# sriramelango/optimized-diffusion-model

Hardware: AMD Instinct MI355X
Metric: trajectories/sec (1000-step PC sampler, NCSN++ [1,9,9], bs=128/GPU) (higher is better)
Workload: dtype f32; 1 GPU; NCSN++ nf=64 ch_mult=[1,2,2] on [128,1,9,9] per GPU, 1000-step reflected PC sampler (predictor euler_maruyama, corrector none), classifier-free guidance on (2B-sample forwards), fp32; global_batch=128, num_scales=1000, score_evals_per_traj=999, parallelism=single GPU

## Files before the change

optimized-diffusion-model_amd/csrc/misc_kernels.h:

```cpp
#pragma once
#include "common.h"

struct PackJob {
    const float* src;
    float* dst;
    int Cin, Cout;
    int Kpad;
    int Npad;
    int n_off;
    int ntap;
    long s_co, s_ci, s_t;
    int kind;
    const float* src2;
    int col_il;
};

__global__ __launch_bounds__(RDMI_THREADS) void pack_kernel(const PackJob* __restrict__ jobs) {
    const PackJob j = jobs[blockIdx.y];
    const int stride = gridDim.x * RDMI_THREADS;
    if (j.kind == 1) {
        for (int i = blockIdx.x * RDMI_THREADS + threadIdx.x; i < j.Cout; i += stride) j.dst[j.n_off + i] = j.src[i];
        return;
    }
    if (j.kind == 4) {
        for (int i = blockIdx.x * RDMI_THREADS + threadIdx.x; i < j.Cout; i += stride) {
            float acc = 0.f;
            for (int k = 0; k < j.Cin; ++k) acc = fmaf(j.src[k], j.src2[(long)k * j.Cout + i], acc);
            j.dst[j.n_off + i] = acc;
        }
        return;
    }
    if (j.kind == 2) {
        const int ncol = (j.Cout + 15) & ~15;
        bf16_t* d16 = reinterpret_cast<bf16_t*>(j.dst);
        const long total = (long)j.ntap * (j.Kpad >> 5) * ncol * 32;
        for (long i = blockIdx.x * RDMI_THREADS + threadIdx.x; i < total; i += stride) {
            const int kk = (int)(i & 31);
            long r = i >> 5;
            const int co = (int)(r % ncol); r /= ncol;
            const int ch = (int)(r % (j.Kpad >> 5));
            const int t = (int)(r / (j.Kpad >> 5));
            const int ci = ch * 32 + kk;
            float v = 0.f;
            if (co < j.Cout && ci < j.Cin) v = j.src[co * j.s_co + ci * j.s_ci + t * j.s_t];
            int pos = j.n_off + co;
            if (j.col_il > 1) { const int F = j.col_il, w = pos % (16 * F); pos = pos - w + (w % F) * 16 + w / F; }
            d16[(((long)t * (j.Kpad >> 5) + ch) * j.Npad + pos) * 32 + kk] = f2bf(v);
        }
        return;
    }
    const int ncol = (j.Cout + 15) & ~15;
    const long total = (long)j.ntap * (j.Kpad >> 4) * ncol * 16;
    for (long i = blockIdx.x * RDMI_THREADS + threadIdx.x; i < total; i += stride) {
        const int kk = (int)(i & 15);
        long r = i >> 4;
        const int co = (int)(r % ncol); r /= ncol;
        const int ch = (int)(r % (j.Kpad >> 4));
        const int t = (int)(r / (j.Kpad >> 4));
        const int ci = ch * 16 + kk;
        float v = 0.f;
        if (co < j.Cout && ci < j.Cin) {
            if (j.kind == 3) {
                for (int k = 0; k < j.Cout; ++k) v = fmaf(j.src[(long)ci * j.s_ci + k * j.s_co], j.src2[(long)k * j.Cout + co], v);
            } else if (j.kind == 5) {
                const int py = t >> 3, px = (t >> 2) & 1, ty = (t >> 1) & 1, tx = t & 1;
                const int ky0 = ty * (1 + py), ky1 = ky0 + 1 + (py != ty);
                const int kx0 = tx * (1 + px), kx1 = kx0 + 1 + (px != tx);
                const float* const s = j.src + co * j.s_co + ci * j.s_ci;
                bool first = true;
                for (int ky = ky0; ky < ky1; ++ky)
                    for (int kx = kx0; kx < kx1; ++kx) {
                        const float wv = s[(ky * 3 + kx) * j.s_t];
                        v = first ? wv : v + wv;
                        first = false;
                    }
            } else v = j.src[co * j.s_co + ci * j.s_ci + t * j.s_t];
        }
        j.dst[(((long)t * (j.Kpad >> 4) + ch) * j.Npad + j.n_off + co) * 16 + kk] = v;
    }
}

struct LinArgs {
    const float* X; int ldx;
    const float* W; int Npad;
    const float* bias;
    float* Y; int ldy;
    int M, N, K;
    int pre;
    const float* fourW; int nfour; int x_mod; int t_is_time; float smin, ratio;
    int use_scalar; float t_scalar;
    const float* labels; const float* Wl; const float* bl; int ncls; int label_rows;
    int row_div;
};

__device__ __forceinline__ float sigma_of(float v, int t_is_time, float smin, float ratio) {
    return t_is_time ? smin * powf(ratio, v) : v;
}

template <int NT, int UNR = 4>
__global__ __launch_bounds__(RDMI_THREADS) void linear_mfma_kernel(LinArgs a) {
    const int tid = threadIdx.x, lane = tid & 63, wave = tid >> 6;
    const int lrow = lane & 15, kq = lane >> 4;
    const int row = blockIdx.x * 16 + lrow;
    int col[NT], lcol[NT];
#pragma unroll
    for (int t = 0; t < NT; ++t) {
        col[t] = blockIdx.y * (64 * NT) + (wave * NT + t) * 16 + lrow;
        lcol[t] = min(col[t], a.Npad - 16 + lrow);
    }
    f32x4 acc[NT];
#pragma unroll
    for (int t = 0; t < NT; ++t) acc[t] = f32x4{0.f, 0.f, 0.f, 0.f};
    float ls = 0.f;
    if (a.pre == 2 && row < a.M) ls = logf(sigma_of(a.use_scalar ? a.t_scalar : a.X[row % a.x_mod], a.t_is_time, a.smin, a.ratio));
#pragma unroll UNR
    for (int ch = 0; ch < (a.K >> 4); ++ch) {
// ... 373 lines not shown
```

optimized-diffusion-model_amd/csrc/rdmi.hip:

```cpp
#include <hip/hip_runtime.h>

#include <algorithm>
#include <cmath>
#include <cstdarg>
#include <cstdio>
#include <cstdlib>
#include <cstring>
#include <climits>
#include <map>
#include <memory>
#include <stdexcept>
#include <string>
#include <vector>

#include "../../include/rdmi.h"
#include "attn_kernel.h"
#include "conv_kernel.h"
#include "misc_kernels.h"
#include "unet_kernel.h"
#include "bwd_kernels.h"
#include "opt_kernels.h"
#include "ode_kernels.h"
#include "tiled_kernels.h"

// ... 246 lines not shown
    L.mid_ch = in_ch;
    std::vector<int> sk(L.skip_ch.rbegin(), L.skip_ch.rend());
    int u = 0, k = 0;
    for (int i = a.n_levels - 1; i >= 0; --i) {
        const int out_ch = a.nf * a.ch_mult[i];
        for (int j = 0; j < a.num_res_blocks + 1; ++j) {
            L.up.push_back({"up_blocks." + std::to_string(u), in_ch + sk[k++], out_ch, (a.attn_levels >> i & 1) != 0, i});
            in_ch = out_ch;
            ++u;
        }
    }
    return L;
}

void build_params(rdmi_ctx* c, const Layout& L) {
    const rdmi_arch& a = c->arch;
    add_param(c, "time_embed.W", {a.nf});
    add_param(c, "time_mlp.0.weight", {c->temb, 2 * a.nf});
    add_param(c, "time_mlp.0.bias", {c->temb});
    add_param(c, "time_mlp.2.weight", {c->temb, c->temb});
    add_param(c, "time_mlp.2.bias", {c->temb});
    if (a.conditional) {
        add_param(c, "label_emb.weight", {c->temb, a.num_classes});
        add_param(c, "label_emb.bias", {c->temb});
    }
    add_conv_p(c, "input_conv", a.channels, a.nf);
    for (auto& b : L.down) add_resblock_p(c, b.name, b.cin, b.cout);
    for (size_t i = 0; i < L.down.size(); ++i)
        if (L.down[i].attn) add_attn_p(c, "down_attn." + std::to_string(i), L.down[i].cout);
    {
        int ch = a.nf;
        for (int i = 0; i < a.n_levels; ++i) {
            ch = a.nf * a.ch_mult[i];
            if (i != a.n_levels - 1) add_conv_p(c, "downsample." + std::to_string(i) + ".Conv_0", ch, ch);
        }
    }
    add_resblock_p(c, "mid_block1", L.mid_ch, L.mid_ch);
    add_resblock_p(c, "mid_block2", L.mid_ch, L.mid_ch);
    for (auto& b : L.up) add_resblock_p(c, b.name, b.cin, b.cout);
    for (size_t i = 0; i < L.up.size(); ++i)
        if (L.up[i].attn) add_attn_p(c, "up_attn." + std::to_string(i), L.up[i].cout);
    for (int k = 0, i = a.n_levels - 1; i >= 1; --i, ++k) {
        const int ch = a.nf * a.ch_mult[i];
        add_conv_p(c, "upsample." + std::to_string(k) + ".Conv_0", ch, ch);
    }
    add_gn(c, "out_norm", a.nf * a.ch_mult[0]);
    add_conv_p(c, "out_conv", a.nf * a.ch_mult[0], a.channels);
}

inline bool up_fold_shape_ok(int Hs, int Ws, int Cin, int Cout) {
    return std::getenv("RDMI_NO_UP_FOLD") == nullptr && Hs * Ws == 16 && Cin == Cout && Cin % 128 == 0;
}

struct Builder {
    rdmi_ctx* c;
    std::vector<int> ints;
    size_t wf = 0;

    int new_tensor(const std::string& name, int C, int H, int W) {
        Tensor t;
        t.name = name; t.C = C; t.H = H; t.W = W;
        t.def = (int)c->ops.size();
        c->tensors.push_back(t);
        return (int)c->tensors.size() - 1;
    }
    void use(int t) { if (t >= 0) c->tensors[t].last = (int)c->ops.size(); }

    size_t alloc_w(size_t n) { size_t o = wf; wf += (n + 63) & ~(size_t)63; return o; }

    void job_pack(const std::string& pname, size_t dst_off, int Cin, int Cout, int Kpad, int Npad, int n_off, int ntap,
                  long s_co, long s_ci, long s_t) {
        PackJob j{};
        j.dst = reinterpret_cast<float*>(dst_off);
        j.Cin = Cin; j.Cout = Cout; j.Kpad = Kpad; j.Npad = Npad; j.n_off = n_off; j.ntap = ntap;
        j.s_co = s_co; j.s_ci = s_ci; j.s_t = s_t; j.kind = 0;
        c->jobs.push_back(j);
        c->job_param.push_back(c->pindex.at(pname));
    }
    void job_copy(const std::string& pname, size_t dst_off, int n, int n_off) {
        PackJob j{};
        j.dst = reinterpret_cast<float*>(dst_off);
        j.Cout = n; j.n_off = n_off; j.kind = 1;
        c->jobs.push_back(j);
        c->job_param.push_back(c->pindex.at(pname));
    }
    size_t pack_conv(const std::string& pre, int cin, int cout) {
        const int Kp = pad16(cin), Np = pad16(cout);
        size_t o = alloc_w((size_t)9 * Kp * Np);
        job_pack(pre + ".weight", o, cin, cout, Kp, Np, 0, 9, (long)cin * 9, 9, 1);
        c->wmap[pre] = o;
        return o;
    }
    size_t pack_nin(const std::string& pre, int cin, int cout) {
        const int Kp = pad16(cin), Np = pad16(cout);
        size_t o = alloc_w((size_t)Kp * Np);
        job_pack(pre + ".W", o, cin, cout, Kp, Np, 0, 1, 1, cout, 0);
        c->wmap[pre] = o;
        return o;
    }

    static std::vector<int> nearest_map(int Hs, int Ws, int Hd, int Wd) {
        std::vector<int> m((size_t)Hd * Wd);
        for (int y = 0; y < Hd; ++y)
            for (int x = 0; x < Wd; ++x) {
                int sy = std::min((int)std::floor(y * ((float)Hs / Hd)), Hs - 1);
                int sx = std::min((int)std::floor(x * ((float)Ws / Wd)), Ws - 1);
// ... 67 lines not shown
    }

    int add_attn(const std::string& name, int tin, int C, int H, int W, int* err) {
        Op op;
        op.kind = OP_ATTN;
        op.name = name;
        if (C != 64 || H * W > 96) { *err = fail("attention %s: only C=64, H*W<=96 is built (got C=%d, L=%d)", name.c_str(), C, H * W); return -1; }
        AttnArgs& a = op.attn;
        a.L = H * W; a.Lpad = pad16(a.L); a.G = std::min(C / 4, 32);
        a.eps = 1e-6f; a.scale = 1.0f / std::sqrt((float)C); a.out_scale = (float)(1.0 / std::sqrt(2.0));
        op.tA = tin;
        op.w_off = alloc_w((size_t)3 * C * C);
        for (int i = 0; i < 3; ++i) {
            PackJob j{};
            j.dst = reinterpret_cast<float*>(op.w_off + (size_t)i * C * C);
            j.Cin = C; j.Cout = C; j.Kpad = C; j.Npad = C; j.n_off = 0; j.ntap = 1; j.s_co = 1; j.s_ci = C; j.s_t = 0; j.kind = 0;
            c->jobs.push_back(j);
            c->job_param.push_back(c->pindex.at(name + ".NIN_" + std::to_string(i) + ".W"));
        }
        c->wmap[name + ".qkv"] = op.w_off;
        {
            const size_t o3 = alloc_w((size_t)3 * C * C);
            for (int i = 0; i < 3; ++i) {
                PackJob j{};
                j.dst = reinterpret_cast<float*>(o3);
                j.Cin = C; j.Cout = C; j.Kpad = C; j.Npad = 3 * C; j.n_off = i * C; j.ntap = 1; j.s_co = 1; j.s_ci = C; j.s_t = 0; j.kind = 0;
                c->jobs.push_back(j);
                c->job_param.push_back(c->pindex.at(name + ".NIN_" + std::to_string(i) + ".W"));
            }
            c->wmap[name + ".qkv3"] = o3;
        }
        {
            const size_t o3 = alloc_w((size_t)3 * C * C);
            for (int i = 0; i < 3; ++i) {
                PackJob j{};
                j.dst = reinterpret_cast<float*>(o3);
                j.Cin = C; j.Cout = C; j.Kpad = C; j.Npad = 3 * C; j.n_off = i * C; j.ntap = 1; j.s_co = 1; j.s_ci = C; j.s_t = 0; j.kind = i == 2 ? 3 : 0;
                c->jobs.push_back(j);
                c->job_param.push_back(c->pindex.at(name + ".NIN_" + std::to_string(i) + ".W"));
                c->job_param2.resize(c->jobs.size(), -1);
                if (i == 2) c->job_param2.back() = c->pindex.at(name + ".NIN_3.W");
            }
            c->wmap[name + ".qkv3f"] = o3;
            const size_t ob = alloc_w((size_t)3 * C);
            c->wmap[name + ".bqkvf"] = ob;
            for (int i = 0; i < 2; ++i) job_copy(name + ".NIN_" + std::to_string(i) + ".b", ob, C, i * C);
            PackJob j{};
            j.dst = reinterpret_cast<float*>(ob);
            j.Cin = C; j.Cout = C; j.n_off = 2 * C; j.kind = 4;
            c->jobs.push_back(j);
            c->job_param.push_back(c->pindex.at(name + ".NIN_2.b"));
            c->job_param2.resize(c->jobs.size(), -1);
            c->job_param2.back() = c->pindex.at(name + ".NIN_3.W");
        }
        op.bqkv_off = alloc_w((size_t)3 * C);
        c->wmap[name + ".bqkv"] = op.bqkv_off;
        for (int i = 0; i < 3; ++i) job_copy(name + ".NIN_" + std::to_string(i) + ".b", op.bqkv_off, C, i * C);
        op.w3_off = pack_nin(name + ".NIN_3", C, C);
        op.p_b3 = name + ".NIN_3.b";
        op.p_gamma = name + ".GroupNorm_0.weight"; op.p_beta = name + ".GroupNorm_0.bias";
        op.flops_per_sample = 2.0 * (4.0 * a.L * C * C + 2.0 * a.L * a.L * C);
        op.attn_C = C; op.attn_H = H; op.attn_W = W;
        use(tin);
        const int out = new_tensor(name, C, H, W);
        op.out_tensor = out;
        c->ops.push_back(op);
        return out;
    }
};

int add_resblock(Builder& b, const std::string& name, int tA, int tB, int CA, int CB, int Ha, int Wa, int H, int W,
                 int cout, int dense_off, int* err) {
    ConvSpec s0;
    s0.name = name + ".Conv_0";
    s0.tA = tA; s0.tB = tB; s0.CA = CA; s0.CB = CB; s0.Ha = Ha; s0.Wa = Wa; s0.Hv = H; s0.Wv = W;
    s0.gn = name + ".GroupNorm_0"; s0.conv = name + ".Conv_0";
    s0.Ho = H; s0.Wo = W; s0.Cout = cout; s0.dense_off = dense_off;
    const int h1 = b.add_conv(s0, err);
    if (*err) return -1;
    ConvSpec s1;
    s1.name = name;
    s1.tA = h1; s1.CA = cout; s1.Ha = H; s1.Wa = W; s1.Hv = H; s1.Wv = W;
    s1.gn = name + ".GroupNorm_1"; s1.conv = name + ".Conv_1";
    s1.Ho = H; s1.Wo = W; s1.Cout = cout;
    s1.scale = (float)(1.0 / std::sqrt(2.0));
    s1.dropout = true;
    if (CA + CB != cout) {
        s1.tScA = tA; s1.tScB = tB; s1.CscA = CA; s1.CscB = CB; s1.Hsa = Ha; s1.Wsa = Wa; s1.nin = name + ".NIN_0";
    } else {
        if (tB >= 0 || Ha != H || Wa != W) { *err = fail("%s: identity shortcut over a gathered input is not built", name.c_str()); return -1; }
        s1.tRes = tA;
    }
    return b.add_conv(s1, err);
}


struct TiledBuilder {
    rdmi_ctx* c; Builder& b;
    size_t top = 0;
    struct TT { size_t off = 0; int C = 0, H = 0, W = 0; bool valid = false; size_t cs = (size_t)-1; int tiles = 0, tile_px = 0; bool bf = false; bool raw16 = false; };
    TT talloc(int C, int H, int W) { TT t; t.off = top; t.C = C; t.H = H; t.W = W; t.valid = true; top += ((size_t)C * H * W + 63) & ~(size_t)63; return t; }
    static int pad32(int a) { return (a + 31) & ~31; }

    bool bf16() const { return c->arch.compute_dtype == 1; }
    size_t pack3x3(const std::string& pre, int cin, int cout) {
        const int Kp = pad32(cin), Np = pad16(cout);
// ... 810 lines not shown
        o.rows = 4 * in.hw(); o.mtiles = 4; o.Cout = Cout; o.Cout_pad = pad16(Cout);
        o.ntap = 4; o.hw_shift = shift_of(o.rows);
        o.main_ph.lds_off = in.off; o.main_ph.rs = in.rs; o.main_ph.nch = in.C / 16;
        for (int t = 0; t < 4; ++t) o.tab_off[t] = up4_table(in.H, in.W, t);
        o.w_tile_stride = 4 * in.C * o.Cout_pad * (int)sizeof(float);
        o.dst_off = dst->off; o.dst_rs = dst->rs;
        if (o.main_ph.nch % 8 != 0 || o.rows <= 4 || o.dst_kind != 0 || in.C != Cout || in.hw() != 16 || in.pm || cur_samp < 0 || dst->C != Cout || dst->hw() != o.rows)
            fail_("folded upsample conv: unsupported shape (" + std::to_string(in.H) + "x" + std::to_string(in.W) + " source, " + std::to_string(in.C) + " -> " + std::to_string(Cout) + " channels)");
        dst->pm = true;
        const int idx = emit(o);
        patch_arena(idx, F_W, c->wmap.at(wkey + ".up4"));
        patch_param(idx, F_BIAS, bias_param);
        return idx;
    }
};

FusedBuilder::LT fused_resblock(FusedBuilder& b, const std::string& name, FusedBuilder::LT& xin, int cout, int dense_off) {
    using LT = FusedBuilder::LT;
    const int H = xin.H, W = xin.W;
    const float rs2 = (float)(1.0 / std::sqrt(2.0));
    if (xin.C != cout) {
        LT out = b.talloc(cout, H, W);
        b.conv(xin, H, W, H, W, 1, 0, 1, name + ".NIN_0", 0, cout, name + ".NIN_0.b", 0, 0, &out, 1.f, -1, nullptr, nullptr, "", "");
        b.gn(xin, name + ".GroupNorm_0", true);
        LT h1 = b.talloc(cout, H, W);
        b.conv(xin, H, W, H, W, 1, 1, 9, name + ".Conv_0", 0, cout, name + ".Conv_0.bias", 0, 0, &h1, 1.f, dense_off, nullptr, nullptr, "", "");
        b.tfree(xin);
        b.gn(h1, name + ".GroupNorm_1", true);
        b.conv(h1, H, W, H, W, 1, 1, 9, name + ".Conv_1", 0, cout, name + ".Conv_1.bias", 0, 0, &out, rs2, -1, &out, nullptr, "", "");
        b.tfree(h1);
        return out;
    }
    LT xact = b.talloc(xin.C, H, W);
    b.gn(xact, name + ".GroupNorm_0", true, &xin);
    LT h1 = b.talloc(cout, H, W);
    b.conv(xact, H, W, H, W, 1, 1, 9, name + ".Conv_0", 0, cout, name + ".Conv_0.bias", 0, 0, &h1, 1.f, dense_off, nullptr, nullptr, "", "");
    b.tfree(xact);
    b.gn(h1, name + ".GroupNorm_1", true);
    LT out = b.talloc(cout, H, W);
    b.conv(h1, H, W, H, W, 1, 1, 9, name + ".Conv_1", 0, cout, name + ".Conv_1.bias", 0, 0, &out, rs2, -1, &xin, nullptr, "", "");
    b.tfree(h1);
    b.tfree(xin);
    return out;
}

FusedBuilder::LT fused_attn(FusedBuilder& b, const std::string& name, FusedBuilder::LT& x) {
    using LT = FusedBuilder::LT;
    rdmi_ctx* c = b.c;
    const int C = x.C, H = x.H, W = x.W, L = H * W, Lpad = pad16(L);
    if (C != 64 || Lpad > 96) { b.fail_("attention: only C=64, H*W<=96 is built"); return x; }
    if (b.cur_samp < 0) { b.fail_("attention inside the multi-sample (low-resolution) section is not built"); return x; }
    LT xn = b.talloc(C, H, W);
    b.gn(xn, name + ".GroupNorm_0", false, &x);
    LT q = b.talloc(C, H, W), k = b.talloc(C, H, W);
    const int ps = Lpad + 4;
    const int vt_bytes = C * ps * 4, p_bytes = L * ps * 4;
    const int vt_off = b.alloc_top(vt_bytes);
    const bool fold3 = !b.train && std::getenv("RDMI_NO_ATTN_FOLD") == nullptr;
    const size_t bq = c->wmap.at(name + (fold3 ? ".bqkvf" : ".bqkv"));
    {
        const int idx = b.conv(xn, H, W, H, W, 1, 0, 1, name + (fold3 ? ".qkv3f" : ".qkv3"), 0, 3 * C, "", bq, 3, &q, 1.f, -1, nullptr, nullptr, "", "");
        FOp& o = b.prog.fprog[(size_t)idx];
        o.dst2_off = k.off; o.dst3_off = vt_off; o.dst3_rs = ps; o.split_C = C;
        o.qkv1 = (std::getenv("RDMI_NO_QKV1") == nullptr && o.ntap == 1 && o.main_ph.nch == 4 && o.Cout_pad == 192 && C == 64 && o.mtiles <= 6) ? 1 : 0;
    }
    b.tfree(xn);
    const int p_off = b.alloc_top(p_bytes);
    LT o = b.talloc(C, H, W);
    {
        FOp a = b.blank(FOP_ATTN);
        a.q_off = q.off; a.k_off = k.off; a.qk_rs = q.rs; a.vt_off = vt_off; a.p_off = p_off; a.ps = ps;
        a.L = L; a.Lpad = Lpad; a.C = C; a.att_scale = 1.0f / std::sqrt((float)C);
        a.dst_off = o.off; a.dst_rs = o.rs;
        if (fold3) { a.resid_off = x.off; a.resid_rs = x.rs; a.scale = (float)(1.0 / std::sqrt(2.0)); }
        const int ia = b.emit(a);
        if (fold3) b.patch_param(ia, FusedBuilder::F_BIAS, name + ".NIN_3.b");
    }
    b.tfree(q); b.tfree(k);
    b.free_bytes(vt_off, vt_bytes); b.free_bytes(p_off, p_bytes);
    if (fold3) { b.tfree(x); return o; }
    LT out = b.talloc(C, H, W);
    b.conv(o, H, W, H, W, 1, 0, 1, name + ".NIN_3", 0, C, name + ".NIN_3.b", 0, 0, &out, (float)(1.0 / std::sqrt(2.0)), -1, &x, nullptr, "", "");
    b.tfree(o);
    b.tfree(x);
    return out;
}

int build_fused_program_pass(rdmi_ctx* c, rdmi_ctx::FusedProg& q, int S, int TAB_RESERVE, int TAB1_RESERVE, int* tab_used, int* tab1_used, bool coop, bool train);

int build_one_program(rdmi_ctx* c, int S, bool coop = false, bool train = false) {
    int used = 0, used1 = 0;
    {
        rdmi_ctx::FusedProg sizing;
        if (int e = build_fused_program_pass(c, sizing, S, 8 * 1024, 24 * 1024, &used, &used1, coop, train)) return e;
    }
    rdmi_ctx::FusedProg q;
    if (int e = build_fused_program_pass(c, q, S, (used + 63) & ~63, (used1 + 63) & ~63, &used, &used1, coop, train)) return e;
    c->progs.push_back(std::move(q));
    return 0;
}

int resident_workgroups() {
#ifdef RDMI_EMU
    return 256;
#else
    int dev = 0, cus = 0;
    if (hipGetDevice(&dev) != hipSuccess || hipDeviceGetAttribute(&cus, hipDeviceAttributeMultiprocessorCount, dev) != hipSuccess) return 0;
    return cus;
#endif
}

int build_fused_program(rdmi_ctx* c) {
    if (int e = build_one_program(c, 1)) return e;
    const char* only = std::getenv("RDMI_S");
    if (const char* e = std::getenv("RDMI_S_MIN_WG")) c->s_min_wg = std::max(1, atoi(e));
    for (int S : {2, 4})
        if (c->progs[0].ok && c->arch.n_levels >= 2 && c->max_batch >= c->s_min_wg * S && (!only || atoi(only) >= S))
            if (int e = build_one_program(c, S)) return e;
    if (const char* e = std::getenv("RDMI_COOP")) c->use_coop = atoi(e) != 0;
#ifdef RDMI_EMU
    c->coop_stride = 1;
#endif
    if (const char* e = std::getenv("RDMI_COOP_STRIDE")) c->coop_stride = std::max(1, atoi(e));
    if (c->progs[0].ok && c->use_coop && c->arch.n_levels >= 2 && !only)
        if (int e = build_one_program(c, 4, true)) return e;
    return 0;
}

int build_fused_program_pass(rdmi_ctx* c, rdmi_ctx::FusedProg& q, int S, int TAB_RESERVE, int TAB1_RESERVE, int* tab_used, int* tab1_used, bool coop, bool train) {
    using LT = FusedBuilder::LT;
    const rdmi_arch& a = c->arch;
// ... 1295 lines not shown
```

optimized-diffusion-model_amd/csrc/unet_kernel.h:

```cpp
#pragma once
#include <cstddef>

#include "common.h"

#define UW_THREADS 512
#define UW_WAVES 8
#ifndef UW_PF_M4
#define UW_PF_M4 4
#endif
#ifndef UW_PF_N1
#define UW_PF_N1 4
#endif
#ifndef UW_PF_KS1
#define UW_PF_KS1 4
#endif
#ifndef UW_PRIO
#define UW_PRIO 0
#endif
#ifndef UW_LIGHT_BARRIER
#define UW_LIGHT_BARRIER 0
#endif

__device__ __forceinline__ void lds_barrier() {
#if defined(__HIP_DEVICE_COMPILE__) && UW_LIGHT_BARRIER
    asm volatile("s_waitcnt lgkmcnt(0)\n\ts_barrier" ::: "memory");
#else
    __syncthreads();
#endif
}

enum { FOP_GATHER = 0, FOP_STORE = 1, FOP_GN = 2, FOP_CONV = 3, FOP_ATTN = 4, FOP_LOADTAB = 5, FOP_XCHG = 6 };

struct FPhase {
    int lds_off;
    int rs;
    int nch;
    int tab_off;
    const float* w;
};

struct FOp {
    int kind;
    int dst_off, dst_rs, rows, C;
    int CA, CB;
    int a_off, a_rs, a_hw, a_mod, a_map_off;
    int b_off, b_rs;
    const float* a_g; const float* b_g;
    float* g_out;
    int G, act; float eps;
    int src_off, src_rs;
    int logT, Cg, magic_c4n, magic_Cg; float inv_cnt;
    int logG;
    const float* gamma; const float* beta;
    int ntap; int tab_off[9];
    FPhase main_ph;
    int nsc; FPhase sc[2];
    int mtiles, Cout, Cout_pad;
    const float* bias; const float* bias2;
    int dense_off;
    int resid_off, resid_rs;
    float scale;
    int dst_kind;
    int dst2_off, dst3_off, dst3_rs, split_C;
    int q_off, k_off, vt_off, p_off, qk_rs, ps;
    int L, Lpad; float att_scale;
    int gn_off, gn_rs, gn_act, gn_raw, gn_slot_off, gn_nslots;
    int samp, hw_shift;
    int qkv1;
    int coop;
    int a_mstride;
    int xidx;
    float* stash;
    int stash_bf16;
    int drop_op;
    int w_tile_stride;
};

struct UnetArgs {
    const FOp* prog; int nops;
    const short* tabs; int tab_bytes;
    int tab_base;
    int zero_off;
    int zero_bytes;
    const float* dense; int dense_stride;
    const float* x_in; int x_mod;
    float* out;
    int NB;
    int S;
    int dbg;
    long long* stamps;
    int coop, coop_stride;
    unsigned long long* xbuf;
    int xslot;
    unsigned epoch_base;
    int out_elems;
    float drop_p; const unsigned long long* seed_dev;
    int* coop_err;
    int coop_break;
};

struct OpW { int w0, w1; };
static_assert(sizeof(FOp) <= 512, "FOp must fit two VGPRs per wave");
__device__ __forceinline__ int opw_at(const OpW& r, int word) {
    return word < 64 ? __builtin_amdgcn_readlane(r.w0, word) : __builtin_amdgcn_readlane(r.w1, word - 64);
}
#define OPI(r, field) opw_at(r, (int)(offsetof(FOp, field) / 4))
#define OPF(r, field) __builtin_bit_cast(float, OPI(r, field))
#define OPP(r, T, field) \
    reinterpret_cast<T*>((unsigned long long)(unsigned)opw_at(r, (int)(offsetof(FOp, field) / 4)) | ((unsigned long long)(unsigned)opw_at(r, (int)(offsetof(FOp, field) / 4) + 1) << 32))
__device__ __forceinline__ OpW opw_load(const FOp* op, int lane) {
    OpW r;
    constexpr int NW = (int)(sizeof(FOp) / 4);
    const int* g = reinterpret_cast<const int*>(op);
    r.w0 = lane < NW ? __builtin_bit_cast(int, ldg1(reinterpret_cast<const float*>(g + lane))) : 0;
    r.w1 = lane + 64 < NW ? __builtin_bit_cast(int, ldg1(reinterpret_cast<const float*>(g + lane + 64))) : 0;
    return r;
}

__device__ __forceinline__ float* lds_f(int off) { return reinterpret_cast<float*>(rdmi_lds + off); }

__device__ __forceinline__ int samp_of(int samp, int hw_shift, int row) { return samp >= 0 ? samp : (row >> hw_shift); }

template <bool MS>
__device__ __forceinline__ void fop_gather(const OpW& w, const UnetArgs& u, int n0, int ncap, int member, int tid) {
    struct { int C, rows, dst_off, dst_rs, CA, CB, a_off, a_rs, a_hw, a_mod, a_map_off, b_off, b_rs, samp, hw_shift; const float* a_g; const float* b_g; } o;
    o.C = OPI(w, C); o.rows = OPI(w, rows); o.dst_off = OPI(w, dst_off); o.dst_rs = OPI(w, dst_rs); o.CA = OPI(w, CA); o.CB = OPI(w, CB);
    o.a_off = OPI(w, a_off); o.a_rs = OPI(w, a_rs); o.a_hw = OPI(w, a_hw); o.a_mod = OPI(w, a_mod); o.a_map_off = OPI(w, a_map_off);
    if (MS && o.a_off >= 0) o.a_off += member * OPI(w, a_mstride);
// ... 623 lines not shown
}

template <bool MS, bool TR = false>
__device__ __forceinline__ void fconv_gn_apply(const OpW& w, const UnetArgs& u, int n0, int mt0, int WM, int nt, int nmt, int lane, float gmul, float gadd, const f32x4 (&acc)[4],
                                               const float (&ps1)[4], const float (&ps2)[4]) {
    const int lrow = lane & 15, kq = lane >> 4;
    const int o_rows = OPI(w, rows), o_Cout = OPI(w, Cout), nslots = OPI(w, gn_nslots);
    const int o_samp = MS ? OPI(w, samp) : 0, hw_shift = MS ? OPI(w, hw_shift) : 0;
    const int col = nt * 16 + lrow;
    const int gcol = min(col, o_Cout - 1) >> 2, G4 = o_Cout >> 2;
    const float* slots = lds_f(OPI(w, gn_slot_off));
    const float inv_cnt = OPF(w, inv_cnt), eps = OPF(w, eps);
    const int act = OPI(w, gn_act), rs = OPI(w, gn_rs);
    float* dstp = lds_f(OPI(w, gn_off));
    float mean = 0.f, rstd = 0.f;
    if (o_samp >= 0) {
        const float* slot = slots + (size_t)gcol * nslots * 2;
        float s1 = 0.f, s2 = 0.f;
        for (int k = 0; k < nslots; k += 2) {
            const f32x4 p = *reinterpret_cast<const f32x4*>(slot + 2 * k);
            s1 += p[0]; s2 += p[1]; s1 += p[2]; s2 += p[3];
        }
        mean = s1 * inv_cnt;
        rstd = (1.0f / sqrtf(fmaxf(s2 * inv_cnt - mean * mean, 0.f) + eps)) * gmul;
    }
#pragma unroll
    for (int i = 0; i < 4; ++i)
        if (i < nmt) {
            if (o_samp < 0) {
                float s1, s2;
                if (hw_shift == 4) {
                    const float* slot = slots + (size_t)((mt0 + i * WM) * G4 + gcol) * 8;
                    const f32x4 p = *reinterpret_cast<const f32x4*>(slot), q = *reinterpret_cast<const f32x4*>(slot + 4);
                    s1 = (p[0] + p[2]) + (q[0] + q[2]); s2 = (p[1] + p[3]) + (q[1] + q[3]);
                } else { s1 = ps1[i]; s2 = ps2[i]; }
                mean = s1 * inv_cnt;
                rstd = (1.0f / sqrtf(fmaxf(s2 * inv_cnt - mean * mean, 0.f) + eps)) * gmul;
            }
            const int row0 = (mt0 + i * WM) * 16 + kq * 4;
#pragma unroll
            for (int r = 0; r < 4; ++r) {
                const float y = (acc[i][r] - mean) * rstd + gadd;
                float ya = act ? silu_f(y) : y;
                if (TR) {
                    const int dop = OPI(w, drop_op);
                    if (dop >= 0 && u.drop_p > 0.f)
                        ya *= dropout_scale((uint64_t)*u.seed_dev, (uint32_t)dop, ((uint64_t)min(n0, u.NB - 1) * o_rows + (row0 + r)) * o_Cout + col, u.drop_p);
                }
                if (row0 + r < o_rows && col < o_Cout) dstp[(row0 + r) * rs + col] = ya;
            }
        }
}

__device__ __forceinline__ void fconv_qkv(const OpW& w, const UnetArgs& u, int wave, int lane) {
    const int lrow = lane & 15, kq = lane >> 4;
    const int wn = wave & 3, wm = wave >> 2;
    const int o_rows = OPI(w, rows), mtiles = OPI(w, mtiles), o_Cout_pad = OPI(w, Cout_pad);
    const int m_lds = OPI(w, main_ph.lds_off), m_rs = OPI(w, main_ph.rs);
    const float* m_w = OPP(w, const float, main_ph.w);
    const float* o_bias = OPP(w, const float, bias);
    const float o_scale = OPF(w, scale);
    const int sc_ = OPI(w, split_C), o_dst = OPI(w, dst_off), o_dst2 = OPI(w, dst2_off), o_dst3 = OPI(w, dst3_off), o_dst_rs = OPI(w, dst_rs), rs3 = OPI(w, dst3_rs);
    const short* tab = reinterpret_cast<const short*>(rdmi_lds + opw_at(w, (int)(offsetof(FOp, tab_off) / 4)));
    const size_t bstride = (size_t)o_Cout_pad * 16;
    f32x4 bf[3][4];
    float add[3];
#pragma unroll
    for (int c = 0; c < 3; ++c) {
        const int col = (wn + 4 * c) * 16 + lrow;
        add[c] = ldg1(o_bias + col);
#pragma unroll
        for (int ch = 0; ch < 4; ++ch) bf[c][ch] = ldg4(m_w + (size_t)col * 16 + kq * 4 + (size_t)ch * bstride);
    }
    int abase[3];
#pragma unroll
    for (int i = 0; i < 3; ++i) abase[i] = arow(tab, min((wm + 2 * i) * 16 + lrow, mtiles * 16 - 1), m_lds, m_rs, u.zero_off) + kq * 16;
    f32x4 acc[3][3];
#pragma unroll
    for (int i = 0; i < 3; ++i)
#pragma unroll
        for (int c = 0; c < 3; ++c) acc[i][c] = f32x4{0.f, 0.f, 0.f, 0.f};
#pragma unroll
    for (int ch = 0; ch < 4; ++ch) {
        f32x4 af[3];
#pragma unroll
        for (int i = 0; i < 3; ++i) af[i] = *reinterpret_cast<const f32x4*>(rdmi_lds + abase[i] + ch * 64);
#pragma unroll
        for (int j = 0; j < 4; ++j)
#pragma unroll
            for (int i = 0; i < 3; ++i)
#pragma unroll
                for (int c = 0; c < 3; ++c) acc[i][c] = mfma16(af[i][j], bf[c][ch][j], acc[i][c]);
    }
    const int lc = wn * 16 + lrow;
    (void)sc_;
#pragma unroll
    for (int i = 0; i < 3; ++i) {
        const int mt = wm + 2 * i;
        if (mt >= mtiles) continue;
        const int row0 = mt * 16 + kq * 4;
#pragma unroll
        for (int c = 0; c < 2; ++c) {
            float* dstp = lds_f(c == 0 ? o_dst : o_dst2);
#pragma unroll
            for (int r = 0; r < 4; ++r)
                if (row0 + r < o_rows) dstp[(row0 + r) * o_dst_rs + lc] = (acc[i][c][r] + add[c]) * o_scale;
        }
        f32x4 v = acc[i][2];
        for (int r = 0; r < 4; ++r) v[r] = (v[r] + add[2]) * o_scale;
        *reinterpret_cast<f32x4*>(lds_f(o_dst3) + lc * rs3 + row0) = v;
    }
}

template <bool DIAG, bool MS, bool TR = false>
__device__ __forceinline__ void fop_conv(const OpW& w, const UnetArgs& u, int n0, int wave, int lane, long long* fine) {
    const int ntiles = OPI(w, Cout_pad) >> 4, mtiles = OPI(w, mtiles);
    const int lWN = (ntiles >= 8 && (ntiles & 7) == 0) ? 3 : (ntiles >= 4 ? 2 : (ntiles >= 2 ? 1 : 0));
    const int WN = 1 << lWN, WM = UW_WAVES >> lWN, lWM = 3 - lWN;
    const int wn = wave & (WN - 1), wm = wave >> lWN;
    const int o_Cout = OPI(w, Cout), o_dense = OPI(w, dense_off);
    const float* o_bias = OPP(w, const float, bias); const float* o_bias2 = OPP(w, const float, bias2);
    if (OPI(w, dst_kind) == 3 && OPI(w, qkv1)) { fconv_qkv(w, u, wave, lane); return; }
    const bool fused_gn = OPI(w, dst_kind) == 0 && OPI(w, gn_off) >= 0;
    const int wts = OPI(w, w_tile_stride);
    const int o_samp = MS ? OPI(w, samp) : 0, hw_shift = MS ? OPI(w, hw_shift) : 0;
    const float* dense_base = u.dense + (size_t)max(o_dense, 0);
    f32x4 acc[4];
    float ps1[4] = {0.f, 0.f, 0.f, 0.f}, ps2[4] = {0.f, 0.f, 0.f, 0.f};
    const int wcol = min(wn * 16 + (lane & 15), o_Cout - 1);
    float gmul = ldg1((fused_gn ? OPP(w, const float, gamma) : o_bias) + wcol), gadd = ldg1((fused_gn ? OPP(w, const float, beta) : o_bias) + wcol);
    int k_mt0 = 0, k_nt = 0, k_nmt = 0;
    for (int nt = wn; nt < ntiles; nt += WN) {
        const int col = nt * 16 + (lane & 15), colc = min(col, o_Cout - 1);
        float add1 = ldg1(o_bias + colc), add2 = ldg1((o_bias2 ? o_bias2 : o_bias) + colc);
        for (int mt0 = wm; mt0 < mtiles; mt0 += wts ? WM : 4 * WM) {
            const int left = (mtiles - mt0 + WM - 1) >> lWM;
            const int nmt = wts ? 1 : (left >= 4 ? 4 : left);
            float daddm[4] = {0.f, 0.f, 0.f, 0.f};
            float dv = ldg1(dense_base + (o_dense >= 0 ? (size_t)min(n0 + max(o_samp, 0), u.NB - 1) * u.dense_stride + colc : 0));
            if (MS && o_dense >= 0 && o_samp < 0) {
#pragma unroll
                for (int i = 0; i < 4; ++i)
                    if (i < nmt) {
                        const int sl = ((mt0 + i * WM) * 16 + (lane >> 4) * 4) >> hw_shift;
                        daddm[i] = ldg1(dense_base + (size_t)min(n0 + sl, u.NB - 1) * u.dense_stride + colc);
                    }
            }
            const bool tapm = (OPI(w, main_ph.nch) & 3) == 0;
            const bool tapm8 = (OPI(w, main_ph.nch) & 7) == 0;
            switch (nmt) {
                case 1:
                    if (OPI(w, rows) <= 4 && OPI(w, dst_kind) != 1 && OPI(w, dst_kind) != 3) {
                        if (tapm8) fconv_main_t<DIAG, 1, false, 8, true>(w, u, mt0, WM, nt, lane, fine, acc);
                        else fconv_main<DIAG, 1, UW_PF_M4, true>(w, u, mt0, WM, nt, lane, fine, acc);
                    } else if (tapm8) fconv_main_t<DIAG, 1, false, 8>(w, u, mt0, WM, nt, lane, fine, acc, (unsigned)mt0 * (unsigned)wts);
                    else if (tapm) fconv_main_t<DIAG, 1>(w, u, mt0, WM, nt, lane, fine, acc);
                    else fconv_main<DIAG, 1, UW_PF_N1>(w, u, mt0, WM, nt, lane, fine, acc);
                    break;
                case 2: fconv_main<DIAG, 2, 8>(w, u, mt0, WM, nt, lane, fine, acc); break;
                case 3: {
                    const int last_rows = OPI(w, rows) - (mt0 + 2 * WM) * 16;
                    const bool lm4 = last_rows >= 1 && last_rows <= 4 && OPI(w, dst_kind) != 1 && OPI(w, dst_kind) != 3;
                    if (tapm) { if (lm4) fconv_main_t<DIAG, 3, true>(w, u, mt0, WM, nt, lane, fine, acc); else fconv_main_t<DIAG, 3>(w, u, mt0, WM, nt, lane, fine, acc); }
                    else if (lm4) fconv_main<DIAG, 3, 4, false, true>(w, u, mt0, WM, nt, lane, fine, acc);
                    else fconv_main<DIAG, 3, 4>(w, u, mt0, WM, nt, lane, fine, acc);
                    break;
                }
                case 4:
                    if (tapm) fconv_main_t<DIAG, 4>(w, u, mt0, WM, nt, lane, fine, acc);
                    else fconv_main<DIAG, 4, 4>(w, u, mt0, WM, nt, lane, fine, acc);
                    break;
                default: break;
            }
            if (DIAG && (u.dbg & 256)) continue;
            use_from_here(add1); use_from_here(add2); use_from_here(dv);
// ... 102 lines not shown
#pragma unroll
    for (int k = 0; k < KMAX; ++k) {
        const int p = tid + k * UW_THREADS;
        if (p < np && !withhold) {
            f32x2 v;
            if (mode == 0) v = *reinterpret_cast<const f32x2*>(lds_f(0) + at(p, m));
            else {
                const int i = p << 1, row = i >> csh, c = i & (Cs - 1);
                v = *reinterpret_cast<const f32x2*>(lds_f(a_off) + row * a_rs + c);
                *reinterpret_cast<f32x2*>(lds_f(0) + at(p, m)) = v;
            }
            const float v0 = v[0], v1 = v[1];
            xbuf_store16(xb, gbase + (unsigned)m * slotb + (unsigned)p * 16u, __builtin_bit_cast(unsigned, v0), __builtin_bit_cast(unsigned, v1), epoch);
        }
    }
    const int nk = (np + UW_THREADS - 1) / UW_THREADS;
    u32x4 y[3 * KMAX];
    unsigned long long spins = 0;
    bool broken = __hip_atomic_load(u.coop_err, __ATOMIC_RELAXED, __HIP_MEMORY_SCOPE_AGENT) != 0;
    if (broken) *failw = 1;
    for (; !broken;) {
#pragma unroll
        for (int k = 0; k < KMAX; ++k)
            if (k < nk) {
                const unsigned po = (unsigned)min(tid + k * UW_THREADS, np - 1) * 16u;
#pragma unroll
                for (int jj = 0; jj < 3; ++jj) y[k * 3 + jj] = xbuf_load16(xb, gbase + (unsigned)((m + 1 + jj) & 3) * slotb + po);
            }
        bool ok = true;
#pragma unroll
        for (int k = 0; k < KMAX; ++k)
            if (k < nk) {
#pragma unroll
                for (int jj = 0; jj < 3; ++jj) { const unsigned t1 = y[k * 3 + jj][1], t3 = y[k * 3 + jj][3]; ok &= t1 == epoch && t3 == epoch; }
            }
        if (ok) break;
        if (++spins > RDMI_SPIN_LIMIT) { *failw = 1; __hip_atomic_store(u.coop_err, 1, __ATOMIC_RELAXED, __HIP_MEMORY_SCOPE_AGENT); break; }
        spin_relax();
    }
#pragma unroll
    for (int k = 0; k < KMAX; ++k) {
        const int p = tid + k * UW_THREADS;
        if (!broken && k < nk && p < np) {
#pragma unroll
            for (int jj = 0; jj < 3; ++jj) {
                const unsigned a = y[k * 3 + jj][0], b = y[k * 3 + jj][2];
                *reinterpret_cast<f32x2*>(lds_f(0) + at(p, (m + 1 + jj) & 3)) = f32x2{__builtin_bit_cast(float, a), __builtin_bit_cast(float, b)};
            }
        }
    }
}

__device__ __forceinline__ void fop_attn(const OpW& w, int wave, int lane) {
    struct { int L, Lpad, q_off, k_off, vt_off, p_off, qk_rs, ps, C, dst_off, dst_rs; float att_scale; } o;
    o.L = OPI(w, L); o.Lpad = OPI(w, Lpad); o.q_off = OPI(w, q_off); o.k_off = OPI(w, k_off); o.vt_off = OPI(w, vt_off); o.p_off = OPI(w, p_off);
    o.qk_rs = OPI(w, qk_rs); o.ps = OPI(w, ps); o.C = OPI(w, C); o.dst_off = OPI(w, dst_off); o.dst_rs = OPI(w, dst_rs); o.att_scale = OPF(w, att_scale);
    const int lrow = lane & 15, kq = lane >> 4;
    const int L = o.L, mtiles = o.Lpad >> 4;
    const float* Q = lds_f(o.q_off);
    const float* K = lds_f(o.k_off);
    const float* Vt = lds_f(o.vt_off);
    float* P = lds_f(o.p_off);
    const int rs = o.qk_rs, ps = o.ps;
    const int nchq = o.C >> 4;
    for (int mt = wave; mt < mtiles; mt += UW_WAVES) {
        f32x4 s[6];
#pragma unroll
        for (int t = 0; t < 6; ++t) s[t] = f32x4{0.f, 0.f, 0.f, 0.f};
        const int qrow = min(mt * 16 + lrow, L - 1);
        for (int ch = 0; ch < nchq; ++ch) {
            const f32x4 af = *reinterpret_cast<const f32x4*>(Q + (size_t)qrow * rs + ch * 16 + kq * 4);
#pragma unroll
            for (int t = 0; t < 6; ++t) {
                if (t < mtiles) {
                    const int krow = min(t * 16 + lrow, L - 1);
                    const f32x4 bf = *reinterpret_cast<const f32x4*>(K + (size_t)krow * rs + ch * 16 + kq * 4);
#pragma unroll
                    for (int j = 0; j < 4; ++j) s[t] = mfma16(af[j], bf[j], s[t]);
                }
            }
        }
#pragma unroll
        for (int r = 0; r < 4; ++r) {
            float mx = -3.0e38f;
#pragma unroll
            for (int t = 0; t < 6; ++t)
                if (t < mtiles && t * 16 + lrow < L) { s[t][r] *= o.att_scale; mx = fmaxf(mx, s[t][r]); }
            mx = row16_max(mx);
            float sum = 0.f;
#pragma unroll
            for (int t = 0; t < 6; ++t)
                if (t < mtiles) {
                    const float e = (t * 16 + lrow < L) ? __expf(s[t][r] - mx) : 0.f;
                    s[t][r] = e;
                    sum += e;
                }
            sum = row16_sum(sum);
            const float inv = 1.0f / sum;
            const int row = mt * 16 + kq * 4 + r;
            if (row < L) {
#pragma unroll
                for (int t = 0; t < 6; ++t)
                    if (t < mtiles) P[(size_t)row * ps + t * 16 + lrow] = s[t][r] * inv;
            }
        }
    }
    lds_barrier();
    {
        const int wn = wave & 3, wm = wave >> 2;
        const int col = wn * 16 + lrow;
        f32x4 acc[3];
#pragma unroll
        for (int i = 0; i < 3; ++i) acc[i] = f32x4{0.f, 0.f, 0.f, 0.f};
        for (int ch = 0; ch < mtiles; ++ch) {
            const f32x4 bf = *reinterpret_cast<const f32x4*>(Vt + (size_t)col * ps + ch * 16 + kq * 4);
#pragma unroll
            for (int i = 0; i < 3; ++i) {
                const int mt = wm + 2 * i;
                if (mt < mtiles) {
                    const int prow = min(mt * 16 + lrow, L - 1);
                    const f32x4 af = *reinterpret_cast<const f32x4*>(P + (size_t)prow * ps + ch * 16 + kq * 4);
#pragma unroll
                    for (int j = 0; j < 4; ++j) acc[i] = mfma16(af[j], bf[j], acc[i]);
                }
            }
        }
        float* O = lds_f(o.dst_off);
        const float* b3 = OPP(w, const float, bias);
        const int o_resid = OPI(w, resid_off), o_resid_rs = OPI(w, resid_rs);
// ... 92 lines not shown
```

Baseline: 182.5 trajectories/s.

## Fold key projection into query weights for attention at C=64

Precomputes W_q·W_k^T (and a matching folded bias) so attention scores become (xn·W_qk)·xn^T. The K projection is dropped and the normalized input is reused directly as K. The fused qkv conv is templated on the number of projections, and in inference it now does only two (folded Q and folded V). This removes one third of the projection MFMAs and one LDS tensor buffer. The cost is an extra precompute pack job and longer lifetime of the normalized input in LDS. It also adds a separate key row stride and relies on the reordered folded weights being numerically equivalent.

```diff
diff --git a/optimized-diffusion-model_amd/csrc/misc_kernels.h b/optimized-diffusion-model_amd/csrc/misc_kernels.h
--- a/optimized-diffusion-model_amd/csrc/misc_kernels.h
+++ b/optimized-diffusion-model_amd/csrc/misc_kernels.h
@@ -26,6 +26,14 @@
         for (int i = blockIdx.x * RDMI_THREADS + threadIdx.x; i < j.Cout; i += stride) {
             float acc = 0.f;
             for (int k = 0; k < j.Cin; ++k) acc = fmaf(j.src[k], j.src2[(long)k * j.Cout + i], acc);
+            j.dst[j.n_off + i] = acc;
+        }
+        return;
+    }
+    if (j.kind == 7) {
+        for (int i = blockIdx.x * RDMI_THREADS + threadIdx.x; i < j.Cin; i += stride) {
+            float acc = 0.f;
+            for (int k = 0; k < j.Cout; ++k) acc = fmaf(j.src[k], j.src2[(long)i * j.Cout + k], acc);
             j.dst[j.n_off + i] = acc;
         }
         return;
@@ -62,6 +70,8 @@
         if (co < j.Cout && ci < j.Cin) {
             if (j.kind == 3) {
                 for (int k = 0; k < j.Cout; ++k) v = fmaf(j.src[(long)ci * j.s_ci + k * j.s_co], j.src2[(long)k * j.Cout + co], v);
+            } else if (j.kind == 6) {
+                for (int k = 0; k < j.Cout; ++k) v = fmaf(j.src[(long)ci * j.s_ci + k * j.s_co], j.src2[(long)co * j.Cout + k], v);
             } else if (j.kind == 5) {
                 const int py = t >> 3, px = (t >> 2) & 1, ty = (t >> 1) & 1, tx = t & 1;
                 const int ky0 = ty * (1 + py), ky1 = ky0 + 1 + (py != ty);
diff --git a/optimized-diffusion-model_amd/csrc/rdmi.hip b/optimized-diffusion-model_amd/csrc/rdmi.hip
--- a/optimized-diffusion-model_amd/csrc/rdmi.hip
+++ b/optimized-diffusion-model_amd/csrc/rdmi.hip
@@ -322,6 +322,10 @@
     return std::getenv("RDMI_NO_UP_FOLD") == nullptr && Hs * Ws == 16 && Cin == Cout && Cin % 128 == 0;
 }
 
+inline bool k_fold_shape_ok(int C, int L) {
+    return std::getenv("RDMI_NO_K_FOLD") == nullptr && std::getenv("RDMI_NO_ATTN_FOLD") == nullptr && std::getenv("RDMI_NO_QKV1") == nullptr && C == 64 && L <= 96;
+}
+
 struct Builder {
     rdmi_ctx* c;
     std::vector<int> ints;
@@ -495,6 +499,27 @@
             c->job_param.push_back(c->pindex.at(name + ".NIN_2.b"));
             c->job_param2.resize(c->jobs.size(), -1);
             c->job_param2.back() = c->pindex.at(name + ".NIN_3.W");
+        }
+        if (k_fold_shape_ok(C, a.L)) {
+            const size_t o2 = alloc_w((size_t)2 * C * C), ob = alloc_w((size_t)2 * C);
+            c->wmap[name + ".qv2f"] = o2;
+            c->wmap[name + ".bqvf"] = ob;
+            for (int i = 0; i < 2; ++i) {
+                PackJob j{};
+                j.dst = reinterpret_cast<float*>(o2);
+                j.Cin = C; j.Cout = C; j.Kpad = C; j.Npad = 2 * C; j.n_off = i * C; j.ntap = 1; j.s_co = 1; j.s_ci = C; j.s_t = 0; j.kind = i == 0 ? 6 : 3;
+                c->jobs.push_back(j);
+                c->job_param.push_back(c->pindex.at(name + (i == 0 ? ".NIN_0.W" : ".NIN_2.W")));
+                c->job_param2.resize(c->jobs.size(), -1);
+                c->job_param2.back() = c->pindex.at(name + (i == 0 ? ".NIN_1.W" : ".NIN_3.W"));
+                PackJob v{};
+                v.dst = reinterpret_cast<float*>(ob);
+                v.Cin = C; v.Cout = C; v.n_off = i * C; v.kind = i == 0 ? 7 : 4;
+                c->jobs.push_back(v);
+                c->job_param.push_back(c->pindex.at(name + (i == 0 ? ".NIN_0.b" : ".NIN_2.b")));
+                c->job_param2.resize(c->jobs.size(), -1);
+                c->job_param2.back() = c->pindex.at(name + (i == 0 ? ".NIN_1.W" : ".NIN_3.W"));
+            }
         }
         op.bqkv_off = alloc_w((size_t)3 * C);
         c->wmap[name + ".bqkv"] = op.bqkv_off;
@@ -1411,31 +1436,35 @@
     if (b.cur_samp < 0) { b.fail_("attention inside the multi-sample (low-resolution) section is not built"); return x; }
     LT xn = b.talloc(C, H, W);
     b.gn(xn, name + ".GroupNorm_0", false, &x);
-    LT q = b.talloc(C, H, W), k = b.talloc(C, H, W);
+    const bool fold3 = !b.train && std::getenv("RDMI_NO_ATTN_FOLD") == nullptr;
+    const bool foldk = fold3 && k_fold_shape_ok(C, L) && c->wmap.count(name + ".qv2f") != 0;
+    const int NP = foldk ? 2 : 3;
+    LT q = b.talloc(C, H, W), k = foldk ? xn : b.talloc(C, H, W);
     const int ps = Lpad + 4;
     const int vt_bytes = C * ps * 4, p_bytes = L * ps * 4;
     const int vt_off = b.alloc_top(vt_bytes);
-    const bool fold3 = !b.train && std::getenv("RDMI_NO_ATTN_FOLD") == nullptr;
-    const size_t bq = c->wmap.at(name + (fold3 ? ".bqkvf" : ".bqkv"));
+    const size_t bq = c->wmap.at(name + (foldk ? ".bqvf" : fold3 ? ".bqkvf" : ".bqkv"));
     {
-        const int idx = b.conv(xn, H, W, H, W, 1, 0, 1, name + (fold3 ? ".qkv3f" : ".qkv3"), 0, 3 * C, "", bq, 3, &q, 1.f, -1, nullptr, nullptr, "", "");
+        const int idx = b.conv(xn, H, W, H, W, 1, 0, 1, name + (foldk ? ".qv2f" : fold3 ? ".qkv3f" : ".qkv3"), 0, NP * C, "", bq, 3, &q, 1.f, -1, nullptr, nullptr, "", "");
         FOp& o = b.prog.fprog[(size_t)idx];
-        o.dst2_off = k.off; o.dst3_off = vt_off; o.dst3_rs = ps; o.split_C = C;
-        o.qkv1 = (std::getenv("RDMI_NO_QKV1") == nullptr && o.ntap == 1 && o.main_ph.nch == 4 && o.Cout_pad == 192 && C == 64 && o.mtiles <= 6) ? 1 : 0;
-    }
-    b.tfree(xn);
+        o.dst2_off = foldk ? q.off : k.off; o.dst3_off = vt_off; o.dst3_rs = ps; o.split_C = C;
+        o.qkv1 = (std::getenv("RDMI_NO_QKV1") == nullptr && (b.train || foldk) && o.ntap == 1 && o.main_ph.nch == 4 && o.Cout_pad == NP * 64 && C == 64 && o.mtiles <= 6) ? 1 : 0;
+        if (foldk && !o.qkv1) b.fail_("attention: the k-folded projection needs the single-pass form");
+    }
+    if (!foldk) b.tfree(xn);
     const int p_off = b.alloc_top(p_bytes);
-    LT o = b.talloc(C, H, W);
+    LT o = foldk ? q : b.talloc(C, H, W);
     {
         FOp a = b.blank(FOP_ATTN);
-        a.q_off = q.off; a.k_off = k.off; a.qk_rs = q.rs; a.vt_off = vt_off; a.p_off = p_off; a.ps = ps;
+        a.q_off = q.off; a.k_off = k.off; a.qk_rs = q.rs; a.k_rs = k.rs; a.vt_off = vt_off; a.p_off = p_off; a.ps = ps;
         a.L = L; a.Lpad = Lpad; a.C = C; a.att_scale = 1.0f / std::sqrt((float)C);
         a.dst_off = o.off; a.dst_rs = o.rs;
         if (fold3) { a.resid_off = x.off; a.resid_rs = x.rs; a.scale = (float)(1.0 / std::sqrt(2.0)); }
         const int ia = b.emit(a);
         if (fold3) b.patch_param(ia, FusedBuilder::F_BIAS, name + ".NIN_3.b");
     }
-    b.tfree(q); b.tfree(k);
+    if (!foldk) b.tfree(q);
+    b.tfree(k);
     b.free_bytes(vt_off, vt_bytes); b.free_bytes(p_off, p_bytes);
     if (fold3) { b.tfree(x); return o; }
     LT out = b.talloc(C, H, W);
diff --git a/optimized-diffusion-model_amd/csrc/unet_kernel.h b/optimized-diffusion-model_amd/csrc/unet_kernel.h
--- a/optimized-diffusion-model_amd/csrc/unet_kernel.h
+++ b/optimized-diffusion-model_amd/csrc/unet_kernel.h
@@ -74,6 +74,7 @@
     int stash_bf16;
     int drop_op;
     int w_tile_stride;
+    int k_rs;
 };
 
 struct UnetArgs {
@@ -803,6 +804,7 @@
         }
 }
 
+template <int NP>
 __device__ __forceinline__ void fconv_qkv(const OpW& w, const UnetArgs& u, int wave, int lane) {
     const int lrow = lane & 15, kq = lane >> 4;
     const int wn = wave & 3, wm = wave >> 2;
@@ -814,51 +816,64 @@
     const int sc_ = OPI(w, split_C), o_dst = OPI(w, dst_off), o_dst2 = OPI(w, dst2_off), o_dst3 = OPI(w, dst3_off), o_dst_rs = OPI(w, dst_rs), rs3 = OPI(w, dst3_rs);
     const short* tab = reinterpret_cast<const short*>(rdmi_lds + opw_at(w, (int)(offsetof(FOp, tab_off) / 4)));
     const size_t bstride = (size_t)o_Cout_pad * 16;
-    f32x4 bf[3][4];
-    float add[3];
-#pragma unroll
-    for (int c = 0; c < 3; ++c) {
+    constexpr int NT1 = NP == 3 ? 3 : 2;
+    f32x4 bf[NP][4];
+    float add[NP];
+#pragma unroll
+    for (int c = 0; c < NP; ++c) {
         const int col = (wn + 4 * c) * 16 + lrow;
         add[c] = ldg1(o_bias + col);
 #pragma unroll
         for (int ch = 0; ch < 4; ++ch) bf[c][ch] = ldg4(m_w + (size_t)col * 16 + kq * 4 + (size_t)ch * bstride);
     }
+    const bool has3 = NP == 3 || wm + 4 < mtiles;
     int abase[3];
 #pragma unroll
     for (int i = 0; i < 3; ++i) abase[i] = arow(tab, min((wm + 2 * i) * 16 + lrow, mtiles * 16 - 1), m_lds, m_rs, u.zero_off) + kq * 16;
-    f32x4 acc[3][3];
+    f32x4 acc[3][NP];
 #pragma unroll
     for (int i = 0; i < 3; ++i)
 #pragma unroll
-        for (int c = 0; c < 3; ++c) acc[i][c] = f32x4{0.f, 0.f, 0.f, 0.f};
+        for (int c = 0; c < NP; ++c) acc[i][c] = f32x4{0.f, 0.f, 0.f, 0.f};
 #pragma unroll
     for (int ch = 0; ch < 4; ++ch) {
-        f32x4 af[3];
-#pragma unroll
-        for (int i = 0; i < 3; ++i) af[i] = *reinterpret_cast<const f32x4*>(rdmi_lds + abase[i] + ch * 64);
+        f32x4 af[NT1];
+#pragma unroll
+        for (int i = 0; i < NT1; ++i) af[i] = *reinterpret_cast<const f32x4*>(rdmi_lds + abase[i] + ch * 64);
 #pragma unroll
         for (int j = 0; j < 4; ++j)
 #pragma unroll
-            for (int i = 0; i < 3; ++i)
-#pragma unroll
-                for (int c = 0; c < 3; ++c) acc[i][c] = mfma16(af[i][j], bf[c][ch][j], acc[i][c]);
+            for (int i = 0; i < NT1; ++i)
+#pragma unroll
+                for (int c = 0; c < NP; ++c) acc[i][c] = mfma16(af[i][j], bf[c][ch][j], acc[i][c]);
+    }
+    if (NP == 2 && has3) {
+        f32x4 af[4];
+#pragma unroll
+        for (int ch = 0; ch < 4; ++ch) af[ch] = *reinterpret_cast<const f32x4*>(rdmi_lds + abase[2] + ch * 64);
+#pragma unroll
+        for (int ch = 0; ch < 4; ++ch)
+#pragma unroll
+            for (int j = 0; j < 4; ++j)
+#pragma unroll
+                for (int c = 0; c < NP; ++c) acc[2][c] = mfma16(af[ch][j], bf[c][ch][j], acc[2][c]);
     }
     const int lc = wn * 16 + lrow;
-    (void)sc_;
+    (void)sc_; (void)o_dst2;
 #pragma unroll
     for (int i = 0; i < 3; ++i) {
         const int mt = wm + 2 * i;
         if (mt >= mtiles) continue;
         const int row0 = mt * 16 + kq * 4;
 #pragma unroll
-        for (int c = 0; c < 2; ++c) {
+        for (int c = 0; c < NP - 1; ++c) {
             float* dstp = lds_f(c == 0 ? o_dst : o_dst2);
 #pragma unroll
             for (int r = 0; r < 4; ++r)
                 if (row0 + r < o_rows) dstp[(row0 + r) * o_dst_rs + lc] = (acc[i][c][r] + add[c]) * o_scale;
         }
-        f32x4 v = acc[i][2];
-        for (int r = 0; r < 4; ++r) v[r] = (v[r] + add[2]) * o_scale;
+        f32x4 v = acc[i][NP - 1];
+        for (int r = 0; r < 4; ++r) v[r] = (v[r] + add[NP - 1]) * o_scale;
         *reinterpret_cast<f32x4*>(lds_f(o_dst3) + lc * rs3 + row0) = v;
     }
 }
@@ -871,7 +886,7 @@
     const int wn = wave & (WN - 1), wm = wave >> lWN;
     const int o_Cout = OPI(w, Cout), o_dense = OPI(w, dense_off);
     const float* o_bias = OPP(w, const float, bias); const float* o_bias2 = OPP(w, const float, bias2);
-    if (OPI(w, dst_kind) == 3 && OPI(w, qkv1)) { fconv_qkv(w, u, wave, lane); return; }
+    if (OPI(w, dst_kind) == 3 && OPI(w, qkv1)) { fconv_qkv<TR ? 3 : 2>(w, u, wave, lane); return; }
     const bool fused_gn = OPI(w, dst_kind) == 0 && OPI(w, gn_off) >= 0;
     const int wts = OPI(w, w_tile_stride);
     const int o_samp = MS ? OPI(w, samp) : 0, hw_shift = MS ? OPI(w, hw_shift) : 0;
@@ -1080,16 +1095,16 @@
 }
 
 __device__ __forceinline__ void fop_attn(const OpW& w, int wave, int lane) {
-    struct { int L, Lpad, q_off, k_off, vt_off, p_off, qk_rs, ps, C, dst_off, dst_rs; float att_scale; } o;
+    struct { int L, Lpad, q_off, k_off, vt_off, p_off, qk_rs, k_rs, ps, C, dst_off, dst_rs; float att_scale; } o;
     o.L = OPI(w, L); o.Lpad = OPI(w, Lpad); o.q_off = OPI(w, q_off); o.k_off = OPI(w, k_off); o.vt_off = OPI(w, vt_off); o.p_off = OPI(w, p_off);
-    o.qk_rs = OPI(w, qk_rs); o.ps = OPI(w, ps); o.C = OPI(w, C); o.dst_off = OPI(w, dst_off); o.dst_rs = OPI(w, dst_rs); o.att_scale = OPF(w, att_scale);
+    o.qk_rs = OPI(w, qk_rs); o.k_rs = OPI(w, k_rs); o.ps = OPI(w, ps); o.C = OPI(w, C); o.dst_off = OPI(w, dst_off); o.dst_rs = OPI(w, dst_rs); o.att_scale = OPF(w, att_scale);
     const int lrow = lane & 15, kq = lane >> 4;
     const int L = o.L, mtiles = o.Lpad >> 4;
     const float* Q = lds_f(o.q_off);
     const float* K = lds_f(o.k_off);
     const float* Vt = lds_f(o.vt_off);
     float* P = lds_f(o.p_off);
-    const int rs = o.qk_rs, ps = o.ps;
+    const int rs = o.qk_rs, krs = o.k_rs, ps = o.ps;
     const int nchq = o.C >> 4;
     for (int mt = wave; mt < mtiles; mt += UW_WAVES) {
         f32x4 s[6];
@@ -1102,7 +1117,7 @@
             for (int t = 0; t < 6; ++t) {
                 if (t < mtiles) {
                     const int krow = min(t * 16 + lrow, L - 1);
-                    const f32x4 bf = *reinterpret_cast<const f32x4*>(K + (size_t)krow * rs + ch * 16 + kq * 4);
+                    const f32x4 bf = *reinterpret_cast<const f32x4*>(K + (size_t)krow * krs + ch * 16 + kq * 4);
 #pragma unroll
                     for (int j = 0; j < 4; ++j) s[t] = mfma16(af[j], bf[j], s[t]);
                 }
```

Result: faster. 184.5 trajectories/s, median of 6 (+1.1%).
